# gaozhitong/MultiShiftSeg

Hardware: AMD Instinct MI355X
Metric: train images/sec (DeepLabV3+ WRN38, fwd + RelContrastiveLoss + bwd + Adam) (higher is better)
Workload: dtype f32; 1 GPU; c3: 2 images (1 orig+aug pair(s)) of 1024x2048 per GPU, stage-2 trainable set, train-mode BN/Dropout2d on the frozen trunk; images_per_gpu=2, height=1024, width=2048, stage=2, parallelism=dp1, rccl_ranks=0, loss_pairing=device, loss_sync=local

## Files before the change

### include/mss_hip.h

```cpp
#ifndef MSS_HIP_H
#define MSS_HIP_H
#include <stdint.h>

#ifdef __cplusplus
extern "C" {
#endif

#define MSS_ABI_VERSION 20
int mss_abi_version(void);

int mss_env_reset(void);

int mss_msda_forward_f32(const float* value, const int64_t* spatial_shapes, const int64_t* level_start_index,
                         const float* sampling_loc, const float* attn_weight, int N, int S, int M, int D, int L,
                         int Lq, int P, float* out, void* stream);
int mss_msda_forward_f64(const double* value, const int64_t* spatial_shapes, const int64_t* level_start_index,
                         const double* sampling_loc, const double* attn_weight, int N, int S, int M, int D, int L,
                         int Lq, int P, double* out, void* stream);
int mss_msda_backward_f32(const float* value, const int64_t* spatial_shapes, const int64_t* level_start_index,
                          const float* sampling_loc, const float* attn_weight, const float* grad_out, int N,
                          int S, int M, int D, int L, int Lq, int P, float* grad_value, float* grad_loc,
                          float* grad_attn, void* stream);
long long mss_msda_backward_workspace_bytes(const int64_t* host_shapes, int N, int M, int D, int L, int Lq, int P);
int mss_msda_backward_binned_f32(const float* value, const int64_t* spatial_shapes, const int64_t* level_start_index,
                                 const int64_t* host_shapes, const float* sampling_loc, const float* attn_weight,
                                 const float* grad_out, int N, int S, int M, int D, int L, int Lq, int P, float* grad_value,
                                 float* grad_loc, float* grad_attn, void* workspace, long long workspace_bytes, void* stream);
int mss_msda_backward_f64(const double* value, const int64_t* spatial_shapes, const int64_t* level_start_index,
                          const double* sampling_loc, const double* attn_weight, const double* grad_out, int N,
                          int S, int M, int D, int L, int Lq, int P, double* grad_value, double* grad_loc,
                          double* grad_attn, void* stream);

int mss_msda_forward_fused_f32(const float* value, const int64_t* spatial_shapes, const int64_t* level_start_index,
                               const float* offsets, const float* logits, const float* reference_points, int N, int S,
                               int M, int D, int L, int Lq, int P, float* out, void* stream);

int mss_msda_prepare_f32(const float* offsets, const float* logits, const float* reference_points,
                         const int64_t* spatial_shapes, int N, int Lq, int M, int L, int P, float* sampling_loc,
                         float* attn_weight, void* stream);
int mss_msda_prepare_backward_ld_f32(const float* attn_weight, const float* grad_attn, const float* grad_loc,
                                     const int64_t* spatial_shapes, int N, int Lq, int M, int L, int P, float* grad_offsets,
                                     long long ld_offsets, float* grad_logits, long long ld_logits, void* stream);
int mss_msda_backward_binned_proj_f32(const float* value, const int64_t* spatial_shapes, const int64_t* level_start_index,
                                      const int64_t* host_shapes, const float* sampling_loc, const float* attn_weight,
                                      const float* grad_out, int N, int S, int M, int D, int L, int Lq, int P, float* grad_value,
                                      float* grad_offsets, long long ld_offsets, float* grad_logits, long long ld_logits,
                                      void* workspace, long long workspace_bytes, void* stream);
int mss_msda_forward_fused_ld_f32(const float* value, const int64_t* spatial_shapes, const int64_t* level_start_index,
                                  const float* offsets, long long ld_offsets, const float* logits, long long ld_logits,
                                  const float* reference_points, int N, int S, int M, int D, int L, int Lq, int P, float* out,
                                  void* stream);
int mss_msda_forward_fused_save_f32(const float* value, const int64_t* spatial_shapes, const int64_t* level_start_index,
                                    const float* offsets, long long ld_offsets, const float* logits, long long ld_logits,
                                    const float* reference_points, int N, int S, int M, int D, int L, int Lq, int P, float* out,
                                    float* sampling_loc_out, float* attn_weight_out, void* stream);
int mss_msda_prepare_ld_f32(const float* offsets, long long ld_offsets, const float* logits, long long ld_logits,
                            const float* reference_points, const int64_t* spatial_shapes, int N, int Lq, int M, int L, int P,
                            float* sampling_loc, float* attn_weight, void* stream);


typedef struct MssConvArgs {
  const float* x;
  const float* w;
  float* y;
  const float* in_scale;
  const float* in_shift;
  const float* out_scale;
  const float* out_shift;
  const float* res;
  int N, H, W, C, ldx;
  int OH, OW, K, Kpad, ldy;
  int R, S, stride, dil, pad;
  int in_ss_stride;
  int in_relu, out_relu;
  int ldres;
  int M, mtiles, ntiles;
  int batch;
  long long x_bs, w_bs, y_bs;
  float* stats;
  int res_mask;
  const void* w_split;
  int route;
  int k_base, k_imgs;
  const int* k_steps;
  long long w_img_stride;
} MssConvArgs;

int mss_conv2d_forward_f32(MssConvArgs* args, void* stream);
int mss_chan_compact_wanted(const MssConvArgs* args);
int mss_chan_compact_index(const float* mask, int N, int C, int* idx, int* place, int* count, int* k_steps, int* col, void* stream);
int mss_chan_compact_act_f32(const float* x, int ldx, float* out, int ldout, int N, int rows_per_image, int C, const int* place,
                             const int* k_steps, const float* scale, const float* shift, void* stream);
int mss_chan_compact_weights_f32(const float* w, float* out, int N, int Kpad, int C, const int* place, const int* k_steps,
                                 void* stream);
int mss_conv2d_kpad(int K);
int mss_conv2d_forward_route(const MssConvArgs* args);
long long mss_gemm_split_weights_bytes(int batch, int Kpad, int C);
int mss_gemm_split_weights_bf16x3(const float* w, void* planes, int batch, int Kpad, int C, long long w_bs, void* stream);
int mss_conv_split_weights_bf16x3(const float* w, void* planes, int taps, int Kpad, int C, void* stream);
int mss_gemm_split_last_mfma(void);
int mss_conv2d_pack_weights_f32(const float* w, float* packed, int K, int C, int R, int S, int Kpad, int Cp,
                                int flip, const int* col, int n_img, int c0, void* stream);
long long mss_conv2d_wgrad_workspace_bytes(const MssConvArgs* args, int Cp);
int mss_conv2d_wgrad_f32(MssConvArgs* args, const float* dy, int lddy, float* dwp, int Cp, float* ws,
                         long long ws_bytes, void* stream);
int mss_conv2d_unpack_wgrad_f32(const float* packed, float* grad, int K, int C, int R, int S, int Kpad,
                                int Cp, int accumulate, const int* place, const int* k_steps, int n_img, int c0, void* stream);
int mss_conv2d_wgrad_route(const MssConvArgs* args, int lddy);

long long mss_wino_num_tiles(int N, int H, int W, int dil, int tile);
int mss_wino_pack_weights_f32(const float* w, float* u, int K, int C, int Kpad, int Cp, int tile, void* stream);
int mss_wino_pack_split_bf16x3(const float* w, void* planes, int K, int C, int Kpad, int tile, void* stream);
int mss_wino_input_transform_f32(const float* x, int ldx, int N, int H, int W, int C, int dil, int tile,
                                 const float* scale, const float* shift, int relu, float* xt, void* stream);
int mss_wino_input_transform_bnbwd_f32(const float* dy, int lddy, const float* x2, int ldx2, int N, int H, int W, int C, int dil,
                                       int tile, const float* scale, const float* shift, const float* mean, const float* invstd,
                                       const double* accum, int relu, float* xt, void* stream);
int mss_wino_input_transform_upcat_f32(const float* a, int lda, int c_split, const float* small, int ld_small, int IH, int IW, int N,
                                       int H, int W, int C, int tile, float* xt, void* stream);
int mss_wino_input_transform_aspp3_f32(const float* x, int ldx, int N, int H, int W, int C, int d, const int* tiles, float* xt0,
                                       float* xt1, float* xt2, void* stream);
int mss_wino_input_transform_aspp3_src2_f32(const float* x0, int ldx0, int C0, const float* scale0, const float* shift0, int ss0,
                                            const float* x1, int ldx1, int C1, const float* scale1, const float* shift1, int ss1,
                                            int N, int H, int W, int d, const int* tiles, float* xt0, float* xt1, float* xt2,
                                            float* sums, float* gap, void* stream);
int mss_wino_input_transform_aspp3_dropped_f32(const float* x0, int ldx0, int C0, const float* scale0, const float* shift0, int ss0,
                                               const float* x1c, int ldx1, int C1, const int* place, const int* k_steps,
                                               int N, int H, int W, int d, const int* tiles, float* xt0, float* xt1, float* xt2,
                                               float* sums, float* gap, void* stream);
int mss_wino_output_transform_f32(const float* yt, int N, int H, int W, int K, int dil, int tile, const float* res,
                                  int ldres, float* y, int ldy, float* stats, void* stream);
int mss_wino_output_stats_parts(int N, int H, int W, int K, int dil, int tile);

int mss_wino_grad_output_transform_f32(const float* dy, int lddy, int N, int H, int W, int K, int dil, int tile,
                                       float* dyt, void* stream);
int mss_wino_weight_grad_transform_f32(const float* du, float* dw, int K, int C, int Kpad, int Cp, int tile,
                                       void* stream);

int mss_nchw_to_nhwc_pad_f32(const float* x, float* y, int N, int C, int H, int W, int Cp, void* stream);
int mss_im2col3x3_c3_f32(const float* img, float* out, int N, int H, int W, void* stream);
int mss_stem_conv_pool_f32(const float* img, const float* w, float* y, int ldy, int N, int H, int W, void* stream);

long long mss_col_reduce_accum_doubles(long long M, int C);
int mss_bn_stats_partials_f32(const float* partials, long long nparts, int C, double* accum, void* stream);
int mss_bn_stats_nhwc_f32(const float* x, long long M, int C, int ldx, double* accum, void* stream);
int mss_bn_finalize_train_f32(const double* accum, long long M, int C, const float* gamma, const float* beta,
                              float eps, float momentum, float* running_mean, float* running_var, float* scale,
                              float* shift, float* save_mean, float* save_invstd, void* stream);
int mss_bn_fold_train_from_partials_f32(const float* partials, long long nparts, int C, double* accum, long long M,
                                        const float* gamma, const float* beta, float eps, float momentum, float* running_mean,
                                        float* running_var, float* scale, float* shift, float* save_mean, float* save_invstd,
                                        void* stream);
int mss_bn_fold_eval_f32(const float* gamma, const float* beta, const float* running_mean,
                         const float* running_var, float eps, int C, float* scale, float* shift, void* stream);
int mss_affine_relu_nhwc_f32(const float* x, int ldx, float* y, int ldy, long long M, int C, const float* scale,
// ... 220 lines not shown
```

### multishiftseg_amd/_lib.py

```python
import ctypes
import os
from ctypes import POINTER, Structure, c_double, c_float, c_int, c_longlong, c_uint32, c_void_p

import torch

_HERE = os.path.dirname(os.path.abspath(__file__))
LIB_PATH = os.environ.get("MSS_LIB", os.path.join(_HERE, "libmss_hip.so"))

MSS_ABI_VERSION = 20
MSS_ERR_BAD_ARG = 1001
MSS_ERR_UNSUPPORTED = 1002


class MssError(RuntimeError):
    pass


MSS_OODM_BATCH = 16


class MssOodmBatch(Structure):
    _fields_ = [("score", c_void_p * MSS_OODM_BATCH), ("label", c_void_p * MSS_OODM_BATCH), ("keys", c_void_p * MSS_OODM_BATCH),
                ("lane_counts", c_void_p * MSS_OODM_BATCH), ("n", ctypes.c_longlong * MSS_OODM_BATCH)]


MSS_M2F_MAX_STEPS = 16


class MssM2fSteps(Structure):
    _fields_ = [("step", c_void_p * MSS_M2F_MAX_STEPS)]


class MssM2fGrads(Structure):
    _fields_ = [("step", c_void_p * MSS_M2F_MAX_STEPS)]


class MssM2fMaps(Structure):
    _fields_ = [("step", c_void_p * MSS_M2F_MAX_STEPS), ("img_stride", c_longlong), ("query_stride", c_longlong), ("pixel_stride", c_longlong),
                ("S", c_int), ("B", c_int), ("Q", c_int), ("h", c_int), ("w", c_int)]


class MssM2fTargets(Structure):
    _fields_ = [("tmask", c_void_p), ("tstart", c_void_p), ("labels", c_void_p), ("total_t", c_int), ("H", c_int), ("W", c_int)]


class MssConvArgs(Structure):
    _fields_ = [
        ("x", c_void_p), ("w", c_void_p), ("y", c_void_p),
        ("in_scale", c_void_p), ("in_shift", c_void_p),
        ("out_scale", c_void_p), ("out_shift", c_void_p),
        ("res", c_void_p),
        ("N", c_int), ("H", c_int), ("W", c_int), ("C", c_int), ("ldx", c_int),
        ("OH", c_int), ("OW", c_int), ("K", c_int), ("Kpad", c_int), ("ldy", c_int),
        ("R", c_int), ("S", c_int), ("stride", c_int), ("dil", c_int), ("pad", c_int),
        ("in_ss_stride", c_int), ("in_relu", c_int), ("out_relu", c_int),
        ("ldres", c_int),
        ("M", c_int), ("mtiles", c_int), ("ntiles", c_int),
        ("batch", c_int), ("x_bs", c_longlong), ("w_bs", c_longlong), ("y_bs", c_longlong),
        ("stats", c_void_p),
        ("res_mask", c_int),
        ("w_split", c_void_p),
        ("route", c_int),
# ... 237 lines not shown
```

### multishiftseg_amd/csrc/conv_igemm.hip

```cpp
#include "mss_epilogue.h"
#include <stdlib.h>

int mss_gemm_nt_dispatch(MssConvArgs p, void* stream);
bool mss_gemm_nt_eligible(const MssConvArgs& p);
bool mss_gemm_few_rows(const MssConvArgs& p);
bool mss_gemm_nt_bf16x3_eligible(const MssConvArgs& p);
bool mss_conv_bf16x3_eligible(const MssConvArgs& p);
int mss_conv_bf16x3_launch(MssConvArgs p, void* stream);
bool mss_wgrad_tn_bf16x3_eligible(const MssConvArgs& p, int lddy);
long long mss_wgrad_tn_bf16x3_ws_bytes(const MssConvArgs& p, int Cp);
int mss_wgrad_tn_bf16x3_launch(const MssConvArgs& p, const float* dy, int lddy, float* dwp, int Cp, float* ws, long long ws_bytes, void* stream);

namespace {

constexpr int NT = 256;

template <int BM, int BN, int BK, int WM, int WN, bool PER_SAMPLE, bool AFFINE>
__global__ __launch_bounds__(NT) void conv_igemm_kernel(MssConvArgs p) {
  constexpr int LDK = BK + 4;
  constexpr int WTM = BM / WM, WTN = BN / WN;
  constexpr int TM = WTM / 32, TN = WTN / 32;
  constexpr int CPR = BK / 4;
  constexpr int RPP = NT / CPR;
  constexpr int A_LD = BM / RPP, B_LD = BN / RPP;
  static_assert(WM * WN == 4, "4 waves per workgroup");
  static_assert(A_LD >= 1 && B_LD >= 1, "tile too small for 256 threads");

  extern __shared__ __attribute__((aligned(16))) float smem[];
  int* live_mask_p = reinterpret_cast<int*>(smem);
  float* As = smem + 4;
  float* Bs = As + 2 * BM * LDK;

  const int tid = threadIdx.x;
  const int lane = tid & 63;
  const int wave = tid >> 6;
  const int wm = wave / WN, wn = wave % WN;

  p.x += (size_t)blockIdx.y * p.x_bs;
  p.w += (size_t)blockIdx.y * p.w_bs;
  p.y += (size_t)blockIdx.y * p.y_bs;
  const int v = mss_xcd_remap(blockIdx.x, gridDim.x);
  const int mt = v / p.ntiles, nt = v % p.ntiles;
  const int m0 = mt * BM, n0 = nt * BN;

  const int chunk = tid % CPR;
  const int row0 = tid / CPR;

  int a_nb[A_LD], a_iy0[A_LD], a_ix0[A_LD], a_n[A_LD];
  const int ohw = p.OH * p.OW;
  int my_live = 0;
  if (tid == 0) *live_mask_p = 0;
#pragma unroll
  for (int j = 0; j < A_LD; ++j) {
// ... 856 lines not shown
WgradPlan wgrad_plan(const MssConvArgs& p) {
  WgradPlan pl;
  pl.ktiles = mss_cdiv(p.K, BKO); pl.ctiles = mss_cdiv(p.C, BCI); pl.taps = p.batch > 1 ? p.batch : p.R * p.S;
  const int base = pl.ktiles * pl.ctiles * pl.taps;
  const int slots = 768;
  int max_splits = mss_cdiv(p.M, BP * 8);
  if (max_splits > 1024) max_splits = 1024;
  if (max_splits < 1) max_splits = 1;
  int splits = 1;
  double best = 0.0;
  for (int sp = 1; sp <= max_splits; ++sp) {
    const long long total = (long long)base * sp;
    const double eff = (double)total / (double)(((total + slots - 1) / slots) * slots);
    if (eff > best + 1e-9) { best = eff; splits = sp; }
    if (eff >= 0.95 && total >= slots) break;
  }
  pl.pps = mss_cdiv(mss_cdiv(p.M, splits), BP) * BP;
  pl.splits = mss_cdiv(p.M, pl.pps);
  return pl;
}

template <int BKO, int BCI, int BP>
long long wgrad_ws_bytes(const MssConvArgs& p, int Cp) {
  const WgradPlan pl = wgrad_plan<BKO, BCI, BP>(p);
  return pl.splits > 1 ? (long long)pl.splits * pl.taps * p.Kpad * Cp * 4 : 0;
}

template <int BKO, int BCI, int BP, int WK>
int launch_wgrad(MssConvArgs& p, const float* dy, int lddy, float* dwp, int Cp, float* ws, long long ws_bytes,
                 hipStream_t stream) {
  const WgradPlan pl = wgrad_plan<BKO, BCI, BP>(p);
  const long long slab = (long long)pl.taps * p.Kpad * Cp;
  if (pl.splits > 1 && (!ws || ws_bytes < (long long)pl.splits * slab * 4)) return MSS_ERR_BAD_ARG;
  const size_t smem = (size_t)2 * BP * (BKO + 4 + BCI + 4) * sizeof(float);
  auto kern = conv_wgrad_kernel<BKO, BCI, BP, WK>;
  hipLaunchKernelGGL(kern, dim3(pl.ktiles * pl.ctiles, pl.taps, pl.splits), dim3(NT), smem, stream, p, dy, lddy,
                     pl.splits > 1 ? ws : dwp, Cp, pl.pps);
  if (pl.splits > 1) {
    launch_wgrad_reduce(ws, dwp, slab / 4, pl.splits, stream);
  }
  return mss_launch_status();
}

typedef float f32x2 __attribute__((ext_vector_type(2)));
__device__ const float tn_zero_row[4096] = {0.f};
template <bool AFFINE = false, bool PERIMG = false>
__global__ __launch_bounds__(256, 1) void gemm_tn_direct_kernel(const float* __restrict__ A, const float* __restrict__ B,
                                                                float* __restrict__ out, int P, int M, int K, int C, long long a_bs,
                                                                long long b_bs, int Kpad, int Cp, int ktiles, int ctiles, int splits,
                                                                int tps, long long total, long long full, float* __restrict__ tail_ws,
                                                                const float* __restrict__ scale = nullptr,
                                                                const float* __restrict__ shift = nullptr, int relu = 0, int lda = 0,
                                                                const int* __restrict__ k_steps = nullptr, int k_base = 0,
                                                                int k_imgs = 1) {
  if (lda <= 0) lda = K;
  constexpr int KB = 4;
  constexpr int TND = 8;
  const int lane = threadIdx.x & 63, wave = threadIdx.x >> 6;
  const long long job = (long long)(PERIMG ? mss_xcd_remap((int)blockIdx.x, (int)gridDim.x) : (int)blockIdx.x) * 4 + wave;
  if (job >= total) return;
  long long t = job;
  int sp = 0, nsp = 1;
  long long tail_tile = -1;
  if (full >= 0) {
    if (job >= full) {
      const long long ntail = (total - full) / splits;
      sp = (int)((job - full) / ntail);
      tail_tile = (job - full) - (long long)sp * ntail;
      t = full + tail_tile;
      nsp = splits;
    }
  } else {
    nsp = splits;
  }
  const int ct = (int)(t % ctiles); t /= ctiles;
  const int kt = (int)(t % ktiles); t /= ktiles;
  int pb;
  if (full >= 0) pb = (int)t;
  else { sp = (int)(t % splits); pb = (int)(t / splits); }
  const int half = lane >> 5, j = lane & 31;
  const int r0 = nsp > 1 ? sp * tps : 0, r1 = nsp > 1 ? (r0 + tps < M ? r0 + tps : M) : M;
  const float* a = A + (size_t)pb * a_bs + (size_t)(kt * (32 * KB) + KB * j);
  const float* b = B + (size_t)pb * b_bs + (size_t)(ct * 128 + 4 * j);
  size_t b_ld = (size_t)C;
  if (PERIMG) {
    const int cend = 16 * (k_base + k_steps[pb % k_imgs]);
    if (ct * 128 >= cend) return;
    if (ct * 128 + 4 * j >= cend) { b = tn_zero_row + 4 * j; b_ld = 0; }
  }
  f32x16 acc[KB][4];
#pragma unroll
  for (int i = 0; i < KB; ++i)
#pragma unroll
    for (int q = 0; q < 4; ++q)
#pragma unroll
      for (int r = 0; r < 16; ++r) acc[i][q][r] = 0.f;
  f32x4 a0[TND], a1[TND];
  f32x4 b0[TND], b1[TND];
  const int last = r1 - 1;
  const float* az = tn_zero_row + (kt * (32 * KB) + KB * j);
  auto fetch = [&](int row, f32x4& va, f32x4& vb) {
    const bool ok = row <= last;
    const size_t rr = (size_t)(ok ? row : last);
    va = *reinterpret_cast<const f32x4*>(ok ? a + rr * lda : az);
    vb = *reinterpret_cast<const f32x4*>(b + rr * (PERIMG ? b_ld : (size_t)C));
  };
  f32x4 sc = {1.f, 1.f, 1.f, 1.f}, sh = {0.f, 0.f, 0.f, 0.f};
  if (AFFINE) {
    if (scale) sc = *reinterpret_cast<const f32x4*>(scale + ct * 128 + 4 * j);
    if (shift) sh = *reinterpret_cast<const f32x4*>(shift + ct * 128 + 4 * j);
  }
  const float fl = relu ? 0.f : -__builtin_huge_valf();
  auto compute = [&](const f32x4 (&va)[TND], const f32x4 (&vb)[TND]) {
#pragma unroll
    for (int d = 0; d < TND; ++d) {
      const f32x4 ca = va[d];
      f32x4 cb = vb[d];
      if (AFFINE) {
        cb = cb * sc + sh;
        cb.x = fmaxf(cb.x, fl); cb.y = fmaxf(cb.y, fl); cb.z = fmaxf(cb.z, fl); cb.w = fmaxf(cb.w, fl);
      }
#pragma unroll
      for (int i = 0; i < KB; ++i)
#pragma unroll
        for (int q = 0; q < 4; ++q) acc[i][q] = __builtin_amdgcn_mfma_f32_32x32x2f32(ca[i], cb[q], acc[i][q], 0, 0, 0);
    }
  };
#pragma unroll
  for (int d = 0; d < TND; ++d) fetch(r0 + 2 * d + half, a0[d], b0[d]);
  for (int r = r0; r < r1; r += 4 * TND) {
#pragma unroll
    for (int d = 0; d < TND; ++d) fetch(r + 2 * TND + 2 * d + half, a1[d], b1[d]);
    __builtin_amdgcn_sched_barrier(0);
    compute(a0, b0);
    __builtin_amdgcn_sched_barrier(0);
#pragma unroll
    for (int d = 0; d < TND; ++d) fetch(r + 4 * TND + 2 * d + half, a0[d], b0[d]);
    __builtin_amdgcn_sched_barrier(0);
    compute(a1, b1);
    __builtin_amdgcn_sched_barrier(0);
  }
  float* o;
  size_t ostride;
  if (tail_tile >= 0) {
    const long long ntail = (total - full) / splits;
    o = tail_ws + ((size_t)sp * ntail + tail_tile) * (128 * 128) + (size_t)(4 * j);
    ostride = 128;
  } else {
    o = out + ((size_t)(full >= 0 ? 0 : sp) * P + pb) * Kpad * Cp + (size_t)(kt * (32 * KB)) * Cp + (size_t)(ct * 128 + 4 * j);
    ostride = Cp;
  }
#pragma unroll
  for (int i = 0; i < KB; ++i)
#pragma unroll
    for (int r = 0; r < 16; ++r) {
      const int m = (r & 3) + 8 * (r >> 2) + 4 * half;
      const f32x4 v = {acc[i][0][r], acc[i][1][r], acc[i][2][r], acc[i][3][r]};
      *reinterpret_cast<f32x4*>(o + (size_t)(KB * m + i) * ostride) = v;
    }
}

__global__ __launch_bounds__(256) void tn_tail_reduce_kernel(const float* __restrict__ tail_ws, float* __restrict__ dwp, long long full,
                                                             long long ntail, int splits, int ktiles, int ctiles, int Kpad, int Cp) {
  const long long ti = blockIdx.x / 16;
  const int part = blockIdx.x % 16;
  long long t = full + ti;
  const int ct = (int)(t % ctiles); t /= ctiles;
  const int kt = (int)(t % ktiles); t /= ktiles;
  const int pb = (int)t;
  const int e = part * 1024 + threadIdx.x * 4;
  const int row = e >> 7, col = e & 127;
  const float* src = tail_ws + (size_t)ti * (128 * 128) + e;
  f32x4 a = *reinterpret_cast<const f32x4*>(src);
  for (int sp = 1; sp < splits; ++sp) a += *reinterpret_cast<const f32x4*>(src + (size_t)sp * ntail * (128 * 128));
  *reinterpret_cast<f32x4*>(dwp + (size_t)pb * Kpad * Cp + (size_t)(kt * 128 + row) * Cp + ct * 128 + col) = a;
}

__device__ float tn_zeros_rt[64];
template <int KB2, bool AFFINE>
__global__ __launch_bounds__(256, 2) void gemm_tn_narrow_kernel(const float* __restrict__ A, int lda, const float* __restrict__ B, int ldb,
                                                                const float* __restrict__ scale, const float* __restrict__ shift,
                                                                int relu, float* __restrict__ out, int M, int K, int Kpad, int Cp,
                                                                int ctiles, int tps, long long total) {
  typedef typename std::conditional<KB2 == 2, f32x2, float>::type avec;
  constexpr int TND = 8;
  const int lane = threadIdx.x & 63, wave = threadIdx.x >> 6;
  const long long job = (long long)blockIdx.x * 4 + wave;
  if (job >= total) return;
  const int ct = (int)(job % ctiles), sp = (int)(job / ctiles);
  const int half = lane >> 5, j = lane & 31;
  const int r0 = sp * tps, r1 = r0 + tps < M ? r0 + tps : M;
  const bool a_ok = KB2 * j + KB2 - 1 < K;
  const float* a = A + KB2 * j;
  const float* b = B + (size_t)(ct * 128 + 4 * j);
  f32x4 sc = {1.f, 1.f, 1.f, 1.f}, sh = {0.f, 0.f, 0.f, 0.f};
  if (AFFINE) {
    if (scale) sc = *reinterpret_cast<const f32x4*>(scale + ct * 128 + 4 * j);
    if (shift) sh = *reinterpret_cast<const f32x4*>(shift + ct * 128 + 4 * j);
  }
  const float fl = relu ? 0.f : -__builtin_huge_valf();
  f32x16 acc[KB2][4];
#pragma unroll
  for (int i = 0; i < KB2; ++i)
#pragma unroll
    for (int q = 0; q < 4; ++q)
#pragma unroll
      for (int r = 0; r < 16; ++r) acc[i][q][r] = 0.f;
  avec a0[TND], a1[TND];
  f32x4 b0[TND], b1[TND];
  const int last = r1 - 1;
  auto fetch = [&](int row, avec& va, f32x4& vb) {
    const bool ok = row <= last;
    const size_t rr = (size_t)(ok ? row : last);
    va = *reinterpret_cast<const avec*>((ok && a_ok) ? a + rr * lda : tn_zeros_rt);
    vb = *reinterpret_cast<const f32x4*>(b + rr * ldb);
  };
  auto compute = [&](const avec (&va)[TND], const f32x4 (&vb)[TND]) {
#pragma unroll
    for (int d = 0; d < TND; ++d) {
      f32x4 cb = vb[d];
      if (AFFINE) {
        cb = cb * sc + sh;
        cb.x = fmaxf(cb.x, fl); cb.y = fmaxf(cb.y, fl); cb.z = fmaxf(cb.z, fl); cb.w = fmaxf(cb.w, fl);
      }
#pragma unroll
      for (int i = 0; i < KB2; ++i) {
        float ai;
        if constexpr (KB2 == 2) ai = va[d][i]; else ai = va[d];
// ... 122 lines not shown
  if (tn_mode() < 5 || p.C % 256) return false;
  const TnPlan w = tn_plan(p, 256, 512);
  const double eff = (double)w.total / (double)(((w.total + 511) / 512) * 512);
  return w.splits == 1 && w.total >= 1024 && eff >= 0.9;
}
inline TnPlan tn_plan_direct(const MssConvArgs& p);
inline TnPlan tn_plan_for(const MssConvArgs& p) { return tn_direct(p) ? tn_plan_direct(p) : tn_wide(p) ? tn_plan(p, 256, 512) : tn_plan(p); }
inline bool tn_direct(const MssConvArgs& p) {
  const int mode = tn_mode();
  if ((mode != 5 && mode != 7) || p.K % 128 || p.C % 128 || p.K > 4096) return false;
  if (mode == 7) return true;
  const TnPlan pl = tn_plan_direct(p);
  return pl.total * 4 >= 1024 * 3;
}
inline TnPlan tn_plan_direct(const MssConvArgs& p) {
  TnPlan pl;
  pl.ktiles = p.K / 128; pl.ctiles = p.C / 128;
  const long long base = (long long)tn_batch(p) * pl.ktiles * pl.ctiles;
  const int slots = 1024;
  int max_splits = mss_cdiv(p.M, 256);
  if (MSS_ENV_INT("MSS_WGRAD_TN_TAIL", 1) != 0 && base > slots && base % slots != 0 &&
      (double)base / (double)(((base + slots - 1) / slots) * slots) < 0.95) {
    const long long tail = base % slots;
    int ts = (int)(slots / tail);
    if (ts > max_splits) ts = max_splits;
    if (ts > 16) ts = 16;
    if (ts >= 2) {
      pl.full = base - tail;
      pl.tps = mss_cdiv(mss_cdiv(p.M, ts), 2) * 2;
      pl.splits = mss_cdiv(p.M, pl.tps);
      pl.total = pl.full + tail * pl.splits;
      return pl;
    }
  }
  const int cap = p.batch > 1 ? 64 : 256;
  if (max_splits > cap) max_splits = cap;
  if (max_splits < 1) max_splits = 1;
  int splits = 1;
  double best = 0.0;
  for (int sp = 1; sp <= max_splits; ++sp) {
    const long long total = base * sp;
    const double eff = (double)total / (double)(((total + slots - 1) / slots) * slots);
    if (eff > best + 1e-9) { best = eff; splits = sp; }
    if (eff >= 0.95 && total >= slots) break;
  }
  pl.tps = mss_cdiv(mss_cdiv(p.M, splits), 2) * 2;
  pl.splits = mss_cdiv(p.M, pl.tps);
  pl.total = base * pl.splits;
  return pl;
}
int launch_wgrad_tn(const MssConvArgs& p, const float* dy, float* dwp, int Cp, float* ws, long long ws_bytes,
                    hipStream_t stream, int lddy = 0) {
  if (p.k_steps) {
    const long long total = (long long)p.batch * (p.K / 128) * (p.C / 128);
    hipLaunchKernelGGL((gemm_tn_direct_kernel<false, true>), dim3((unsigned)((total + 3) / 4)), dim3(256), 0, stream, dy, p.x, dwp, p.batch,
                       p.M, p.K, p.C, p.y_bs, p.x_bs, p.Kpad, Cp, p.K / 128, p.C / 128, 1, p.M, total, -1ll, (float*)nullptr,
                       (const float*)nullptr, (const float*)nullptr, 0, lddy, p.k_steps, p.k_base, p.k_imgs);
    return mss_launch_status();
  }
  if (tn_direct(p)) {
    const TnPlan pl = tn_plan_direct(p);
    const int P = tn_batch(p);
    const long long a_bs = p.batch > 1 ? p.y_bs : 0, b_bs = p.batch > 1 ? p.x_bs : 0;
    const long long slab = (long long)P * p.Kpad * Cp;
    if (pl.full >= 0) {
      const long long ntail = (pl.total - pl.full) / pl.splits;
      if (!ws || ws_bytes < tn_tail_bytes(pl)) return MSS_ERR_BAD_ARG;
      if (p.in_scale || p.in_shift || p.in_relu)
        hipLaunchKernelGGL(gemm_tn_direct_kernel<true>, dim3((unsigned)((pl.total + 3) / 4)), dim3(256), 0, stream, dy, p.x, dwp, P, p.M,
                           p.K, p.C, a_bs, b_bs, p.Kpad, Cp, pl.ktiles, pl.ctiles, pl.splits, pl.tps, pl.total, pl.full, ws, p.in_scale,
                           p.in_shift, p.in_relu, lddy);
      else
        hipLaunchKernelGGL(gemm_tn_direct_kernel<false>, dim3((unsigned)((pl.total + 3) / 4)), dim3(256), 0, stream, dy, p.x, dwp, P, p.M, p.K,
                           p.C, a_bs, b_bs, p.Kpad, Cp, pl.ktiles, pl.ctiles, pl.splits, pl.tps, pl.total, pl.full, ws, (const float*)nullptr,
                           (const float*)nullptr, 0, lddy);
      hipLaunchKernelGGL(tn_tail_reduce_kernel, dim3((unsigned)(ntail * 16)), dim3(256), 0, stream, ws, dwp, pl.full, ntail, pl.splits,
                         pl.ktiles, pl.ctiles, p.Kpad, Cp);
      return mss_launch_status();
    }
    if (pl.splits > 1 && (!ws || ws_bytes < (long long)pl.splits * slab * 4)) return MSS_ERR_BAD_ARG;
    float* out = pl.splits > 1 ? ws : dwp;
    if (p.in_scale || p.in_shift || p.in_relu)
      hipLaunchKernelGGL(gemm_tn_direct_kernel<true>, dim3((unsigned)((pl.total + 3) / 4)), dim3(256), 0, stream, dy, p.x, out, P, p.M,
                         p.K, p.C, a_bs, b_bs, p.Kpad, Cp, pl.ktiles, pl.ctiles, pl.splits, pl.tps, pl.total, -1ll, (float*)nullptr,
                         p.in_scale, p.in_shift, p.in_relu, lddy);
    else
      hipLaunchKernelGGL(gemm_tn_direct_kernel<false>, dim3((unsigned)((pl.total + 3) / 4)), dim3(256), 0, stream, dy, p.x, out, P, p.M, p.K,
                         p.C, a_bs, b_bs, p.Kpad, Cp, pl.ktiles, pl.ctiles, pl.splits, pl.tps, pl.total, -1ll, (float*)nullptr,
                         (const float*)nullptr, (const float*)nullptr, 0, lddy);
    if (pl.splits > 1) {
      launch_wgrad_reduce(ws, dwp, slab / 4, pl.splits, stream);
    }
    return mss_launch_status();
  }
  const bool wide = tn_wide(p);
  const TnPlan pl = tn_plan_for(p);
  const int P = tn_batch(p);
  const long long a_bs = p.batch > 1 ? p.y_bs : 0, b_bs = p.batch > 1 ? p.x_bs : 0;
  const long long slab = (long long)P * p.Kpad * Cp;
  if (pl.splits > 1 && (!ws || ws_bytes < (long long)pl.splits * slab * 4)) return MSS_ERR_BAD_ARG;
  const size_t smem = (size_t)4 * TN_BT * TN_LD * sizeof(float);
  static int per_cu = 0, cus = 256;
  if (per_cu == 0) {
    int dev = 0, n = 0;
    hipDeviceProp_t prop;
    if (hipGetDevice(&dev) == hipSuccess && hipGetDeviceProperties(&prop, dev) == hipSuccess) cus = prop.multiProcessorCount;
    if (hipOccupancyMaxActiveBlocksPerMultiprocessor(&n, gemm_tn_wgrad_kernel, NT, smem) != hipSuccess || n < 1) n = 3;
    per_cu = n > 3 ? 3 : n;
  }
// ... 177 lines not shown
```

### multishiftseg_amd/kernels.py

```python
import ctypes
import os

import torch

from . import _lib
from ._lib import MssConvArgs, call, ptr


class Act:
    __slots__ = ("buf", "N", "H", "W", "C", "ld", "c0", "stats")

    def __init__(self, buf, C=None, c0=0):
        assert buf.dim() == 4 and buf.is_contiguous() and buf.dtype == torch.float32
        self.buf = buf
        self.stats = None
        self.N, self.H, self.W, self.ld = buf.shape
        self.C = self.ld - c0 if C is None else C
        self.c0 = c0
        assert self.c0 % 4 == 0 and self.ld % 4 == 0 and self.c0 + self.C <= self.ld

    @staticmethod
    def empty(N, H, W, C, device, ld=None):
        return Act(torch.empty((N, H, W, ld or C), device=device, dtype=torch.float32), C)

# ... 792 lines not shown
            call("mss_wino_grad_output_transform_f32", dy.ptr, dy.ld, N, H, W, K, dil, ts, ptr(dyt))
        du = torch.empty((P, Kpad, Cp), device=dev, dtype=torch.float32)
        a = MssConvArgs()
        a.x = ptr(xt)
        a.N, a.H, a.W, a.C, a.ldx = 1, 1, T, C, C
        a.OH, a.OW, a.K, a.Kpad = 1, T, K, Kpad
        a.R, a.S, a.stride, a.dil, a.pad = 1, 1, 1, 1, 0
        a.batch, a.x_bs, a.y_bs = P, T * C, T * K
        a.route = 1 if gemm_route() == "bf16x3" else 0
        ws, ws_bytes = _wgrad_workspace(a, Cp, dev)
        with _Timed(_wgrad_kind(a, K), 2.0 * P * T * K * C, (P, 1, T, C, K, 1, 1, 1)):
            call("mss_conv2d_wgrad_f32", ctypes.byref(a), ptr(dyt), K, ptr(du), Cp, ptr(ws), ws_bytes)
        grad = torch.empty((K, C, 3, 3), device=dev, dtype=torch.float32)
        call("mss_wino_weight_grad_transform_f32", ptr(du), ptr(grad), K, C, Kpad, Cp, ts)
    return grad


def aspp_dropped_weights(rows, K, C, Kpad, ld, tile, dropped):
    assert Kpad == K and K % 128 == 0
    N = dropped.N
    wg = torch.empty((N, K, C, 3, 3), device=rows.device, dtype=torch.float32)
    call("mss_conv2d_unpack_wgrad_f32", ptr(rows), ptr(wg), K, C, 3, 3, Kpad, ld, 0, ptr(dropped.place), ptr(dropped.k_steps), N, dropped.C0)
    P = (tile + 2) ** 2
    u = torch.empty((P, N * K, C), device=rows.device, dtype=torch.float32)
    call("mss_wino_pack_weights_f32", ptr(wg), ptr(u), N * K, C, N * K, C, tile)
    return WinoWeight(u, K, C, Kpad, C, tile)


def conv3x3_dropped(x, ww, dil, out, keep_xt, want_stats, xt, dropped):
    N, H, W, C, K = x.N, x.H, x.W, ww.C, ww.K
    with _Timed("conv_winograd", 2.0 * N * H * W * K * C * 9, (N, H, W, C, K, 3, 1, dil)):
        return _wino_gemm_and_output(xt, ww, N, H, W, dil, None, out, keep_xt, want_stats, dropped=dropped)


def conv3x3_wgrad_dropped(x, dy, K, C, dil, xt, dropped):
    N, H, W = x.N, x.H, x.W
    dev = xt.device
    ts = WINO_TILE_OF_P[xt.shape[0]]
    P, T = xt.shape[0], xt.shape[1]
    Ti = T // N
    assert T % N == 0 and dropped.N == N and K % 128 == 0 and C % 128 == 0 and tuple(xt.shape) == (P, T, C)
    with _Timed("wgrad_winograd", 2.0 * N * H * W * K * C * 9, (N, H, W, C, K, 3, 1, dil)):
        dyt = torch.empty((P, T, K), device=dev, dtype=torch.float32)
        with _Timed("wino_transform", 4.0 * (N * H * W * K + P * T * K), ("grad_output", N, H, W, K, dil, ts)):
            call("mss_wino_grad_output_transform_f32", dy.ptr, dy.ld, N, H, W, K, dil, ts, ptr(dyt))
        du = torch.empty((P, N * K, C), device=dev, dtype=torch.float32)
        a = MssConvArgs()
        a.x = ptr(xt)
        a.N, a.H, a.W, a.C, a.ldx = 1, 1, Ti, C, C
        a.OH, a.OW, a.K, a.Kpad = 1, Ti, K, K
        a.R, a.S, a.stride, a.dil, a.pad = 1, 1, 1, 1, 0
        a.batch, a.x_bs, a.y_bs = P * N, Ti * C, Ti * K
        a.k_steps, a.k_base, a.k_imgs = ptr(dropped.k_steps), dropped.C0 // 16, N
        with _Timed("conv_wgrad", 2.0 * P * Ti * K * dropped.columns(), ("aspp_dropped", P, N, Ti, C, K)):
            call("mss_conv2d_wgrad_f32", ctypes.byref(a), ptr(dyt), K, ptr(du), C, None, 0)
        grad = torch.empty((N, K, C, 3, 3), device=dev, dtype=torch.float32)
        call("mss_wino_weight_grad_transform_f32", ptr(du), ptr(grad), N * K, C, N * K, C, ts)
    return grad


def conv3x3_wgrad(x, dy, K, C, dil=1, in_affine=None, in_relu=False, xt=None, max_tile=6):
    tile = WINO_TILE_OF_P[xt.shape[0]] if xt is not None else wino_tile(x.H, x.W, dil, max_tile)
    if use_winograd(C, K, 1, in_affine, tile):
        return conv2d_wgrad_winograd(x, dy, K, C, dil, in_affine, in_relu, xt=xt, tile=tile)
    return conv2d_wgrad(x, dy, K, C, 3, 3, dil=dil, pad=dil, in_affine=in_affine, in_relu=in_relu)


def image_to_nhwc(img, Cp=16):
    n, c, h, w = img.shape
    img = img.contiguous()
    out = Act.empty(n, h, w, Cp, img.device)
    call("mss_nchw_to_nhwc_pad_f32", ptr(img), out.ptr, n, c, h, w, Cp)
    return out


def stem_im2col(img):
    n, c, h, w = img.shape
    if c != 3:
        raise ValueError(f"the stem expects a 3-channel image, got {c}")
    img = img.contiguous()
    out = Act.empty(n, h, w, 32, img.device)
    call("mss_im2col3x3_c3_f32", ptr(img), out.ptr, n, h, w)
    return out


def stem_conv_pool(img, weight):
    n, c, h, w = img.shape
    if c != 3 or tuple(weight.shape) != (64, 3, 3, 3):
        raise ValueError(f"the fused stem expects a 3-channel image and a [64,3,3,3] weight, got {tuple(img.shape)} / {tuple(weight.shape)}")
    img = img.contiguous()
    wt = weight.detach().contiguous()
    out = Act.empty(n, (h - 1) // 2 + 1, (w - 1) // 2 + 1, 64, img.device)
    call("mss_stem_conv_pool_f32", ptr(img), ptr(wt), out.ptr, out.ld, n, h, w)
    return out


def packed_stem(param):
    def make():
        k = param.shape[0]
        w = torch.zeros((k, 32, 1, 1), device=param.device, dtype=torch.float32)
        w[:, :27, 0, 0] = param.detach().reshape(k, 27)
        return pack_weight(w)
    return _cached_pack(param, ("stem",), make)


class BNState:
    __slots__ = ("scale", "shift", "save_mean", "save_invstd", "M", "train")

# ... 910 lines not shown
```

Measured before the change: 22.60 images/s.

## Pack live per-image tiles in dropped-channel TN wgrad and split the tail rows

The per-image TN weight-gradient kernel used to launch one job for every (position, image, ktile, ctile), even for column tiles that are dead because of channel dropout. It now decodes a compact job index that covers only the live ctiles of each image, so workgroups for dropped columns exit right away. When the live count leaves a partial last round of slots, the remaining tiles are split across row ranges into a workspace and summed by a new reduce kernel. This costs a 64MB workspace allocation per call and a plan computation inside every thread block.

Measured after the change: 23.10 images/s (median of 6 runs). 1.02x the previous value.

```diff
diff --git a/include/mss_hip.h b/include/mss_hip.h
--- a/include/mss_hip.h
+++ b/include/mss_hip.h
@@ -6,7 +6,7 @@
 extern "C" {
 #endif
 
-#define MSS_ABI_VERSION 20
+#define MSS_ABI_VERSION 21
 int mss_abi_version(void);
 
 int mss_env_reset(void);
@@ -101,6 +101,7 @@
 int mss_gemm_split_last_mfma(void);
 int mss_conv2d_pack_weights_f32(const float* w, float* packed, int K, int C, int R, int S, int Kpad, int Cp,
                                 int flip, const int* col, int n_img, int c0, void* stream);
+#define MSS_WGRAD_PERIMG_TAIL_BYTES (1024ll * 128 * 128 * 4)
 long long mss_conv2d_wgrad_workspace_bytes(const MssConvArgs* args, int Cp);
 int mss_conv2d_wgrad_f32(MssConvArgs* args, const float* dy, int lddy, float* dwp, int Cp, float* ws,
                          long long ws_bytes, void* stream);
diff --git a/multishiftseg_amd/_lib.py b/multishiftseg_amd/_lib.py
--- a/multishiftseg_amd/_lib.py
+++ b/multishiftseg_amd/_lib.py
@@ -7,7 +7,8 @@
 _HERE = os.path.dirname(os.path.abspath(__file__))
 LIB_PATH = os.environ.get("MSS_LIB", os.path.join(_HERE, "libmss_hip.so"))
 
-MSS_ABI_VERSION = 20
+MSS_ABI_VERSION = 21
+MSS_WGRAD_PERIMG_TAIL_BYTES = 1024 * 128 * 128 * 4
 MSS_ERR_BAD_ARG = 1001
 MSS_ERR_UNSUPPORTED = 1002
 
diff --git a/multishiftseg_amd/csrc/conv_igemm.hip b/multishiftseg_amd/csrc/conv_igemm.hip
--- a/multishiftseg_amd/csrc/conv_igemm.hip
+++ b/multishiftseg_amd/csrc/conv_igemm.hip
@@ -1,4 +1,6 @@
 #include "mss_epilogue.h"
+#include "tn_perimg_plan.h"
+static_assert(MSS_WGRAD_PERIMG_TAIL_BYTES == (long long)TN_PERIMG_MAX_SLOTS * 128 * 128 * 4, "include/mss_hip.h and tn_perimg_plan.h disagree");
 #include <stdlib.h>
 
 int mss_gemm_nt_dispatch(MssConvArgs p, void* stream);
@@ -961,32 +963,45 @@
                                                                 const float* __restrict__ scale = nullptr,
                                                                 const float* __restrict__ shift = nullptr, int relu = 0, int lda = 0,
                                                                 const int* __restrict__ k_steps = nullptr, int k_base = 0,
-                                                                int k_imgs = 1) {
+                                                                int k_imgs = 1, int pi_slots = 0) {
   if (lda <= 0) lda = K;
   constexpr int KB = 4;
   constexpr int TND = 8;
   const int lane = threadIdx.x & 63, wave = threadIdx.x >> 6;
-  const long long job = (long long)(PERIMG ? mss_xcd_remap((int)blockIdx.x, (int)gridDim.x) : (int)blockIdx.x) * 4 + wave;
-  if (job >= total) return;
-  long long t = job;
+  long long t;
   int sp = 0, nsp = 1;
-  long long tail_tile = -1;
-  if (full >= 0) {
-    if (job >= full) {
-      const long long ntail = (total - full) / splits;
-      sp = (int)((job - full) / ntail);
-      tail_tile = (job - full) - (long long)sp * ntail;
-      t = full + tail_tile;
+  long long tail_tile = -1, ntail = 0;
+  int ct, kt, pb;
+  if (PERIMG && pi_slots > 0) {
+    const TnPerimgPlan pl = tn_perimg_plan(P / k_imgs, k_imgs, ktiles, ctiles, k_base, k_steps, pi_slots, M, tail_ws != nullptr);
+    const int nwg = (int)((pl.total + 3) / 4), nrun = pl.tail ? (int)(pl.full / 4) : nwg;
+    const int bid = (int)blockIdx.x;
+    if (bid >= nwg) return;
+    const long long job = (long long)(bid < nrun ? mss_xcd_remap(bid, nrun) : bid) * 4 + __builtin_amdgcn_readfirstlane(wave);
+    TnPerimgJob jb;
+    if (!tn_perimg_decode(pl, k_steps, job, jb)) return;
+    ct = jb.ct; kt = jb.kt; pb = jb.pos * k_imgs + jb.img;
+    if (jb.tail_tile >= 0) { sp = jb.sp; nsp = pl.splits; tail_tile = jb.tail_tile; ntail = pl.tail; tps = pl.tps; }
+  } else {
+    const long long job = (long long)(PERIMG ? mss_xcd_remap((int)blockIdx.x, (int)gridDim.x) : (int)blockIdx.x) * 4 + wave;
+    if (job >= total) return;
+    t = job;
+    if (full >= 0) {
+      if (job >= full) {
+        ntail = (total - full) / splits;
+        sp = (int)((job - full) / ntail);
+        tail_tile = (job - full) - (long long)sp * ntail;
+        t = full + tail_tile;
+        nsp = splits;
+      }
+    } else {
       nsp = splits;
     }
-  } else {
-    nsp = splits;
-  }
-  const int ct = (int)(t % ctiles); t /= ctiles;
-  const int kt = (int)(t % ktiles); t /= ktiles;
-  int pb;
-  if (full >= 0) pb = (int)t;
-  else { sp = (int)(t % splits); pb = (int)(t / splits); }
+    ct = (int)(t % ctiles); t /= ctiles;
+    kt = (int)(t % ktiles); t /= ktiles;
+    if (full >= 0) pb = (int)t;
+    else { sp = (int)(t % splits); pb = (int)(t / splits); }
+  }
   const int half = lane >> 5, j = lane & 31;
   const int r0 = nsp > 1 ? sp * tps : 0, r1 = nsp > 1 ? (r0 + tps < M ? r0 + tps : M) : M;
   const float* a = A + (size_t)pb * a_bs + (size_t)(kt * (32 * KB) + KB * j);
@@ -1052,7 +1067,6 @@
   float* o;
   size_t ostride;
   if (tail_tile >= 0) {
-    const long long ntail = (total - full) / splits;
     o = tail_ws + ((size_t)sp * ntail + tail_tile) * (128 * 128) + (size_t)(4 * j);
     ostride = 128;
   } else {
@@ -1083,6 +1097,24 @@
   f32x4 a = *reinterpret_cast<const f32x4*>(src);
   for (int sp = 1; sp < splits; ++sp) a += *reinterpret_cast<const f32x4*>(src + (size_t)sp * ntail * (128 * 128));
   *reinterpret_cast<f32x4*>(dwp + (size_t)pb * Kpad * Cp + (size_t)(kt * 128 + row) * Cp + ct * 128 + col) = a;
+}
+
+__global__ __launch_bounds__(256) void tn_tail_reduce_perimg_kernel(const float* __restrict__ tail_ws, float* __restrict__ dwp, int P,
+                                                                    int k_imgs, int ktiles, int ctiles, int k_base,
+                                                                    const int* __restrict__ k_steps, int slots, int rows, int Kpad,
+                                                                    int Cp) {
+  const int ti = blockIdx.x / 16, part = blockIdx.x % 16;
+  const TnPerimgPlan pl = tn_perimg_plan(P, k_imgs, ktiles, ctiles, k_base, k_steps, slots, rows, 1);
+  if (ti >= pl.tail) return;
+  TnPerimgJob jb;
+  if (!tn_perimg_decode(pl, k_steps, pl.full + ti, jb)) return;
+  const int pb = jb.pos * k_imgs + jb.img;
+  const int e = part * 1024 + threadIdx.x * 4;
+  const int row = e >> 7, col = e & 127;
+  const float* src = tail_ws + (size_t)ti * (128 * 128) + e;
+  f32x4 a = *reinterpret_cast<const f32x4*>(src);
+  for (int sp = 1; sp < pl.splits; ++sp) a += *reinterpret_cast<const f32x4*>(src + (size_t)sp * pl.tail * (128 * 128));
+  *reinterpret_cast<f32x4*>(dwp + (size_t)pb * Kpad * Cp + (size_t)(jb.kt * 128 + row) * Cp + jb.ct * 128 + col) = a;
 }
 
 __device__ float tn_zeros_rt[64];
@@ -1311,9 +1343,24 @@
 int launch_wgrad_tn(const MssConvArgs& p, const float* dy, float* dwp, int Cp, float* ws, long long ws_bytes,
                     hipStream_t stream, int lddy = 0) {
   if (p.k_steps) {
-    const long long total = (long long)p.batch * (p.K / 128) * (p.C / 128);
-    hipLaunchKernelGGL((gemm_tn_direct_kernel<false, true>), dim3((unsigned)((total + 3) / 4)), dim3(256), 0, stream, dy, p.x, dwp, p.batch,
-                       p.M, p.K, p.C, p.y_bs, p.x_bs, p.Kpad, Cp, p.K / 128, p.C / 128, 1, p.M, total, -1ll, (float*)nullptr,
+    const int ktiles = p.K / 128, ctiles = p.C / 128;
+    const long long worst = (long long)p.batch * ktiles * ctiles;
+    if (MSS_ENV_INT("MSS_WGRAD_PERIMG_PACK", 1) != 0 && p.k_imgs <= TN_PERIMG_MAX_IMGS) {
+      int slots = MSS_ENV_INT("MSS_WGRAD_TN_SLOTS", TN_PERIMG_MAX_SLOTS) / 32 * 32;
+      slots = slots < 32 ? 32 : slots > TN_PERIMG_MAX_SLOTS ? TN_PERIMG_MAX_SLOTS : slots;
+      const int P = p.batch / p.k_imgs;
+      const bool tail = MSS_ENV_INT("MSS_WGRAD_TN_TAIL", 1) != 0 && ws && ws_bytes >= (long long)slots * (128 * 128 * 4) && worst > slots;
+      const long long jobs = tn_perimg_worst_jobs(P, p.k_imgs, ktiles, ctiles, slots, tail);
+      hipLaunchKernelGGL((gemm_tn_direct_kernel<false, true>), dim3((unsigned)((jobs + 3) / 4)), dim3(256), 0, stream, dy, p.x, dwp, p.batch,
+                         p.M, p.K, p.C, p.y_bs, p.x_bs, p.Kpad, Cp, ktiles, ctiles, 1, p.M, jobs, -1ll, tail ? ws : (float*)nullptr,
+                         (const float*)nullptr, (const float*)nullptr, 0, lddy, p.k_steps, p.k_base, p.k_imgs, slots);
+      if (tail)
+        hipLaunchKernelGGL(tn_tail_reduce_perimg_kernel, dim3((unsigned)(slots / 2 * 16)), dim3(256), 0, stream, ws, dwp, P, p.k_imgs, ktiles,
+                           ctiles, p.k_base, p.k_steps, slots, p.M, p.Kpad, Cp);
+      return mss_launch_status();
+    }
+    hipLaunchKernelGGL((gemm_tn_direct_kernel<false, true>), dim3((unsigned)((worst + 3) / 4)), dim3(256), 0, stream, dy, p.x, dwp, p.batch,
+                       p.M, p.K, p.C, p.y_bs, p.x_bs, p.Kpad, Cp, ktiles, ctiles, 1, p.M, worst, -1ll, (float*)nullptr,
                        (const float*)nullptr, (const float*)nullptr, 0, lddy, p.k_steps, p.k_base, p.k_imgs);
     return mss_launch_status();
   }
diff --git a/multishiftseg_amd/csrc/tn_perimg_plan.h b/multishiftseg_amd/csrc/tn_perimg_plan.h
--- /dev/null
+++ b/multishiftseg_amd/csrc/tn_perimg_plan.h
@@ -0,0 +1,86 @@
+#pragma once
+
+#if !defined(__HIPCC__) && !defined(__host__)
+#define __host__
+#define __device__
+#endif
+
+#define TN_PERIMG_MAX_IMGS 64
+#define TN_PERIMG_MAX_SLOTS 1024
+
+struct TnPerimgPlan {
+  int ktiles, ctiles, k_imgs, k_base, rows;
+  int S;
+  long long live;
+  long long full;
+  long long total;
+  int tail;
+  int splits, tps;
+};
+
+struct TnPerimgJob {
+  int pos, img, kt, ct;
+  int sp;
+  int tail_tile;
+  int r0, r1;
+};
+
+__host__ __device__ static inline int tn_perimg_ctiles(int k_base, int k_steps_n, int ctiles) {
+  const int cols = 16 * (k_base + k_steps_n);
+  int L = cols > 0 ? (cols + 127) / 128 : 0;
+  return L < ctiles ? L : ctiles;
+}
+
+__host__ __device__ static inline TnPerimgPlan tn_perimg_plan(int P, int k_imgs, int ktiles, int ctiles, int k_base, const int* k_steps,
+                                                              int slots, int rows, int want_tail) {
+  TnPerimgPlan pl;
+  pl.ktiles = ktiles; pl.ctiles = ctiles; pl.k_imgs = k_imgs; pl.k_base = k_base; pl.rows = rows;
+  int sum = 0;
+  for (int n = 0; n < k_imgs; ++n) sum += tn_perimg_ctiles(k_base, k_steps[n], ctiles);
+  pl.S = ktiles * sum;
+  pl.live = (long long)P * pl.S;
+  pl.full = pl.live; pl.total = pl.live; pl.tail = 0; pl.splits = 1; pl.tps = rows;
+  if (!want_tail || pl.live <= slots || pl.live % slots == 0) return pl;
+  const long long rounds = (pl.live + slots - 1) / slots * slots;
+  if (pl.live * 20 >= rounds * 19) return pl;
+  const int tail = (int)(pl.live % slots);
+  int ts = slots / tail;
+  const int max_splits = (rows + 255) / 256;
+  if (ts > max_splits) ts = max_splits;
+  if (ts > 16) ts = 16;
+  if (ts < 2) return pl;
+  pl.tail = tail;
+  pl.full = pl.live - tail;
+  pl.tps = ((rows + ts - 1) / ts + 1) / 2 * 2;
+  pl.splits = (rows + pl.tps - 1) / pl.tps;
+  pl.total = pl.full + (long long)tail * pl.splits;
+  return pl;
+}
+
+__host__ __device__ static inline bool tn_perimg_decode(const TnPerimgPlan& pl, const int* k_steps, long long job, TnPerimgJob& j) {
+  if (job < 0 || job >= pl.total) return false;
+  long long t = job;
+  j.sp = 0; j.tail_tile = -1;
+  if (job >= pl.full) {
+    j.sp = (int)((job - pl.full) / pl.tail);
+    j.tail_tile = (int)((job - pl.full) - (long long)j.sp * pl.tail);
+    t = pl.full + j.tail_tile;
+  }
+  j.pos = (int)(t / pl.S);
+  int rem = (int)(t - (long long)j.pos * pl.S);
+  j.img = 0; j.kt = 0; j.ct = 0;
+  for (int n = 0; n < pl.k_imgs; ++n) {
+    const int L = tn_perimg_ctiles(pl.k_base, k_steps[n], pl.ctiles);
+    const int g = pl.ktiles * L;
+    if (rem < g) { j.img = n; j.kt = rem / L; j.ct = rem - j.kt * L; break; }
+    rem -= g;
+  }
+  j.r0 = j.tail_tile >= 0 ? j.sp * pl.tps : 0;
+  j.r1 = j.tail_tile >= 0 && j.r0 + pl.tps < pl.rows ? j.r0 + pl.tps : pl.rows;
+  return true;
+}
+
+__host__ __device__ static inline long long tn_perimg_worst_jobs(int P, int k_imgs, int ktiles, int ctiles, int slots, int want_tail) {
+  const long long worst = (long long)P * k_imgs * ktiles * ctiles;
+  return worst + (want_tail && worst > slots ? slots : 0);
+}
diff --git a/multishiftseg_amd/kernels.py b/multishiftseg_amd/kernels.py
--- a/multishiftseg_amd/kernels.py
+++ b/multishiftseg_amd/kernels.py
@@ -868,8 +868,9 @@
         a.R, a.S, a.stride, a.dil, a.pad = 1, 1, 1, 1, 0
         a.batch, a.x_bs, a.y_bs = P * N, Ti * C, Ti * K
         a.k_steps, a.k_base, a.k_imgs = ptr(dropped.k_steps), dropped.C0 // 16, N
+        ws = torch.empty(_lib.MSS_WGRAD_PERIMG_TAIL_BYTES // 4, device=dev, dtype=torch.float32)
         with _Timed("conv_wgrad", 2.0 * P * Ti * K * dropped.columns(), ("aspp_dropped", P, N, Ti, C, K)):
-            call("mss_conv2d_wgrad_f32", ctypes.byref(a), ptr(dyt), K, ptr(du), C, None, 0)
+            call("mss_conv2d_wgrad_f32", ctypes.byref(a), ptr(dyt), K, ptr(du), C, ptr(ws), _lib.MSS_WGRAD_PERIMG_TAIL_BYTES)
         grad = torch.empty((N, K, C, 3, 3), device=dev, dtype=torch.float32)
         call("mss_wino_weight_grad_transform_f32", ptr(du), ptr(grad), N * K, C, N * K, C, ts)
     return grad
```
